# Dokumushikun/jittor-clip-fewshot

Hardware: AMD Instinct MI355X
Metric: images/sec ViT-B/32 fwd+LoRA-bwd bs=256 (higher is better)
Workload: dtype f32; 1 GPU; cfg-2: ViT-B/32 + rank-4 LoRA(q,k,v; 12 text + 12 vision blocks; shipped lora_weights.pkl) + 4 text-prompt tokens; run_lora train step = text tower fwd+bwd on 403 captions + image tower fwd+bwd + 100*cos CE + AdamW; global_batch=256, images_per_rank=256, captions=403, tower_streams=2, text_positions=77, parallelism=dp1

## Files before the change

### include/clipfs.h

```cpp
#ifndef CLIPFS_H
#define CLIPFS_H

#include <stddef.h>
#include <stdint.h>

#ifdef __cplusplus
extern "C" {
#endif

#define CLIPFS_OK 0
#define CLIPFS_EINVAL 1
#define CLIPFS_HIPERR_BASE 1000

#define CLIPFS_ABI_VERSION 2
int clipfs_abi_version(void);
const char* clipfs_source_stamp(void);
const char* clipfs_gemm_source_stamp(void);
const char* clipfs_last_error(void);

typedef struct clipfs_gemm_args {
  size_t struct_size;
  const float* A;
  const float* B;
  float* C;
  int M, N, K;
  int lda, ldb, ldc;
  float alpha;
  const float* bias;
  const float* residual;
  int ldres;
  int act;
  float* aux_out;
  const float* aux_in;
  const float* lora_t;
  const float* lora_b;
  int lora_r, lora_nseg, lora_seg_width;
  float lora_scale;
  int a_mode;
  int img_res, patch, out_tokens;
  const void* B_planes;
  int b_format;
  float* workspace;
  size_t workspace_floats;
  const void* A_f16;
  void* C_f16;
  int aux_f16;
  int* counters;
  size_t counters_ints;
} clipfs_gemm_args;
int clipfs_gemm_nt(const clipfs_gemm_args* args, void* stream);
int clipfs_split_bf16(const float* src, void* planes, size_t n, void* stream);
int clipfs_convert_f16(const float* src, void* dst, size_t n, void* stream);
int clipfs_gemm_splits(int M, int N, int K);
int clipfs_gemm_tile_rows(int M, int N);
#define CLIPFS_F16_64X128 0
#define CLIPFS_F16_64X128_S2 1
#define CLIPFS_F16_128X128 2
#define CLIPFS_F16_256X128 3
#define CLIPFS_F16_PP_REG 4
#define CLIPFS_F16_PP_LDS 5
#define CLIPFS_F16_PH16 6
#define CLIPFS_F16_PH16_WIDE 7
#define CLIPFS_F16_PH32 8
typedef struct clipfs_f16_launch {
  int kernel;
  int m_begin, m_end;
  int side;
} clipfs_f16_launch;
typedef struct clipfs_f16_plan {
  int n;
  clipfs_f16_launch launch[3];
} clipfs_f16_plan;
int clipfs_gemm_f16_plan(const clipfs_gemm_args* args, int cus, clipfs_f16_plan* out);
size_t clipfs_gemm_workspace_floats(int M, int N, int K);
size_t clipfs_gemm_counter_ints(int M, int N, int K);
int clipfs_gemm_timing(int enable);
int clipfs_gemm_timing_collect(double* total_ms, double* total_flops, int* launches);
double clipfs_gemm_timing_last_bytes(void);

int clipfs_layernorm_fwd(const float* x, int ldx, const float* gamma, const float* beta, float* y,
                         float* mean, float* rstd, int rows, int width, float eps, void* stream);
int clipfs_layernorm_bwd(const float* dy, const float* x, int ldx, const float* gamma, const float* mean,
                         const float* rstd, const float* dres, float* dx, int lddx, int rows, int width,
                         void* stream);
int clipfs_layernorm_bwd_rows(const float* dy, const float* x, int ldx, const float* gamma, const float* mean,
                              const float* rstd, const int32_t* xmap, const float* dres, float* dx, int lddx, int rows,
                              int width, void* stream);
int clipfs_layernorm_fwd_f16(const float* x, int ldx, const float* gamma, const float* beta, float* y, void* y16,
                             float* mean, float* rstd, int rows, int width, float eps, void* stream);
int clipfs_layernorm_bwd_f16(const float* dy, const float* x, int ldx, const float* gamma, const float* mean,
                             const float* rstd, const float* dres, float* dx, void* dx16, int lddx, int rows, int width,
                             void* stream);
int clipfs_layernorm_bwd_rows_f16(const float* dy, const float* x, int ldx, const float* gamma, const float* mean,
                                  const float* rstd, const int32_t* xmap, const float* dres, float* dx, void* dx16, int lddx,
                                  int rows, int width, void* stream);
int clipfs_layernorm_fwd_lora_ok(int width, int r, int nseg);
int clipfs_layernorm_fwd_lora(const float* x, int ldx, const float* gamma, const float* beta, float* y, void* y16,
                              float* mean, float* rstd, int rows, int width, float eps, const float* A, float* t, int r,
                              int nseg, unsigned seg_mask, float p, uint64_t seed, uint32_t stream_base, uint32_t drow0,
                              void* keep_bits, void* stream);
int clipfs_layernorm_fwd_lora_map(const float* x, int ldx, const float* gamma, const float* beta, float* y, void* y16,
                                  float* mean, float* rstd, int rows, int width, float eps, const float* A, float* t, int r,
                                  int nseg, unsigned seg_mask, float p, uint64_t seed, uint32_t stream_base, uint32_t drow0,
                                  const int32_t* drow_map, void* keep_bits, void* stream);

int clipfs_attention_fwd(const float* qkv, float* out, float* lse, int batch, int seq, int heads, int causal,
                         void* stream);
// ... 256 lines not shown
```

### jittor-clip-fewshot_amd/clipfs/_lib.py

```python
from __future__ import annotations

import ctypes as C
import os

ABI_VERSION = 2

_HERE = os.path.dirname(os.path.abspath(__file__))
_TAG = os.environ.get("CLIPFS_LIB_TAG", "")
LIB_PATH = os.path.join(_HERE, f"libclipfs_hip_{_TAG}.so" if _TAG else "libclipfs_hip.so")

c_f32p = C.c_void_p
c_stream = C.c_void_p


class ClipfsError(RuntimeError):
    pass


class GemmArgs(C.Structure):
    _fields_ = [
        ("struct_size", C.c_size_t),
        ("A", C.c_void_p), ("B", C.c_void_p), ("C", C.c_void_p),
        ("M", C.c_int), ("N", C.c_int), ("K", C.c_int),
        ("lda", C.c_int), ("ldb", C.c_int), ("ldc", C.c_int),
# ... 39 lines not shown
    _fields_ = [("family", C.c_int), ("groups", C.c_int), ("rq", C.c_int), ("sr_b", C.c_int), ("slices_b", C.c_int),
                ("sr_a", C.c_int), ("slices_a", C.c_int), ("work_floats", C.c_size_t), ("part_a_offset", C.c_size_t),
                ("keep_bits_ok", C.c_int), ("f16dy_ok", C.c_int), ("launches", C.c_int), ("launch", LoraLaunch * 6)]


LORA_OPS = ("down", "bwd", "bwd_f16dy")
LORA_X_ACT, LORA_KEEP_BITS, LORA_FROZEN, LORA_DX = 1, 2, 4, 8
LORA_FAMILIES = ("mfma", "row")

F16_KERNELS = ("64x128", "64x128_s2", "128x128", "256x128", "pp_reg", "pp_lds", "ph16", "ph16_wide", "ph32")


class Block(C.Structure):
    _fields_ = [(n, C.c_void_p) for n in (
        "ln1_g", "ln1_b", "ln2_g", "ln2_b",
        "w_qkv", "b_qkv", "w_qkv_t",
        "w_o", "b_o", "w_o_t",
        "w_fc", "b_fc", "w_fc_t",
        "w_pr", "b_pr", "w_pr_t",
        "lora_a_qkv", "lora_b_qkv", "lora_a_o", "lora_b_o",
        "g_lora_a_qkv", "g_lora_b_qkv", "g_lora_a_o", "g_lora_b_o")] + [("lora_mask", C.c_uint)] + [
        (n, C.c_void_p) for n in ("w_qkv_p", "w_o_p", "w_fc_p", "w_pr_p", "w_qkv_t_p", "w_o_t_p", "w_fc_t_p", "w_pr_t_p",
                                  "g_ln1_b", "g_ln2_b", "g_b_q", "g_b_k", "g_b_v", "g_b_o", "g_b_fc", "g_b_pr",
                                  "lora_a_fc", "lora_b_fc", "lora_a_pr", "lora_b_pr",
                                  "g_lora_a_fc", "g_lora_b_fc", "g_lora_a_pr", "g_lora_b_pr",
                                  "prompt", "g_prompt")] + [("prompt_first", C.c_int), ("prompt_rows", C.c_int)]


class Tower(C.Structure):
    _fields_ = [
        ("struct_size", C.c_size_t), ("block_size", C.c_size_t),
        ("width", C.c_int), ("heads", C.c_int), ("layers", C.c_int), ("seq", C.c_int), ("causal", C.c_int),
        ("lora_r", C.c_int), ("lora_scale", C.c_float), ("lora_dropout", C.c_float),
        ("dropout_seed", C.c_uint64), ("dropout_stream0", C.c_uint32), ("dropout_row0", C.c_uint32),
        ("blocks", C.POINTER(Block)), ("weight_format", C.c_int),
        ("gemm_counters", C.c_void_p), ("gemm_counters_ints", C.c_size_t),
        ("grad_lo", C.c_int),
    ]


_i, _f, _p, _sz = C.c_int, C.c_float, C.c_void_p, C.c_size_t
_u, _u64, _u32 = C.c_uint, C.c_uint64, C.c_uint32

SIGNATURES = {
    "clipfs_abi_version": (_i, []),
    "clipfs_last_error": (C.c_char_p, []),
    "clipfs_source_stamp": (C.c_char_p, []),
    "clipfs_gemm_source_stamp": (C.c_char_p, []),
    "clipfs_gemm_nt": (_i, [C.POINTER(GemmArgs), _p]),
    "clipfs_split_bf16": (_i, [_p, _p, _sz, _p]),
    "clipfs_convert_f16": (_i, [_p, _p, _sz, _p]),
    "clipfs_gemm_splits": (_i, [_i, _i, _i]),
    "clipfs_gemm_tile_rows": (_i, [_i, _i]),
    "clipfs_gemm_f16_plan": (_i, [C.POINTER(GemmArgs), _i, C.POINTER(F16Plan)]),
    "clipfs_gemm_workspace_floats": (_sz, [_i, _i, _i]),
    "clipfs_gemm_counter_ints": (_sz, [_i, _i, _i]),
    "clipfs_gemm_timing": (_i, [_i]),
    "clipfs_gemm_timing_collect": (_i, [C.POINTER(C.c_double), C.POINTER(C.c_double), C.POINTER(C.c_int)]),
    "clipfs_gemm_timing_last_bytes": (C.c_double, []),
    "clipfs_layernorm_fwd": (_i, [_p, _i, _p, _p, _p, _p, _p, _i, _i, _f, _p]),
    "clipfs_layernorm_bwd": (_i, [_p, _p, _i, _p, _p, _p, _p, _p, _i, _i, _i, _p]),
    "clipfs_layernorm_fwd_f16": (_i, [_p, _i, _p, _p, _p, _p, _p, _p, _i, _i, _f, _p]),
    "clipfs_layernorm_fwd_lora_ok": (_i, [_i, _i, _i]),
    "clipfs_layernorm_fwd_lora": (_i, [_p, _i, _p, _p, _p, _p, _p, _p, _i, _i, _f, _p, _p, _i, _i, _u, _f, _u64, _u32, _u32, _p, _p]),
    "clipfs_layernorm_bwd_f16": (_i, [_p, _p, _i, _p, _p, _p, _p, _p, _p, _i, _i, _i, _p]),
    "clipfs_attention_fwd": (_i, [_p, _p, _p, _i, _i, _i, _i, _p]),
    "clipfs_attention_bwd": (_i, [_p, _p, _p, _p, _p, _p, _i, _i, _i, _i, _p]),
    "clipfs_attention_lse_floats": (_sz, [_i, _i, _i]),
    "clipfs_attention_plan": (_i, [_i, _i, _i, _i, _i, _i, C.POINTER(AttentionPlan)]),
    "clipfs_attention_mfma_max_seq": (_i, []),
    "clipfs_attention_mfma_long_fwd": (_i, [_p, _p, _p, _i, _i, _i, _i, _i, _i, _p]),
    "clipfs_attention_mfma_long_bwd": (_i, [_p, _p, _p, _p, _p, _p, _i, _i, _i, _i, _i, _i, _p]),
    "clipfs_attention_f16_max_seq": (_i, []),
    "clipfs_attention_f16_fwd": (_i, [_p, _i, _p, _p, _p, _i, _i, _i, _i, _p]),
    "clipfs_attention_f16_bwd": (_i, [_p, _i, _p, _i, _p, _p, _p, _p, _p, _i, _i, _i, _i, _p]),
    "clipfs_lora_keep_bits_ok": (_i, [_i, _i, _i, _i]),
    "clipfs_lora_plan": (_i, [_i, _i, _i, _i, _i, _i, _i, C.POINTER(LoraPlan)]),
    "clipfs_lora_down": (_i, [_p, _p, _p, _i, _i, _i, _i, _u, _f, _u64, _u32, _u32, _p, _p]),
    "clipfs_lora_bwd_work_floats": (_sz, [_i, _i, _i, _i]),
    "clipfs_lora_bwd": (_i, [_p, _p, _p, _p, _p, _p, _p, _p, _p, _i, _i, _i, _i, _i, _u, _f, _f, _u64, _u32, _u32, _p, _p, _p]),
    "clipfs_lora_bwd_work_floats2": (_sz, [_i, _i, _i, _i, _i]),
    "clipfs_lora_bwd_xact": (_i, [_p, _p, _p, _p, _p, _p, _p, _p, _p, _i, _i, _i, _i, _f, _f, _u64, _u32, _u32, _i, _p, _p]),
    "clipfs_gelu_bwd_inplace": (_i, [_p, _p, _sz, _p]),
    "clipfs_lora_bwd_f16dy_ok": (_i, [_i, _i, _i, _i]),
    "clipfs_lora_bwd_f16dy": (_i, [_p, _p, _p, _p, _p, _p, _p, _p, _p, _i, _i, _i, _i, _i, _u, _f, _f, _u64, _u32, _u32, _p, _p, _p]),
    "clipfs_vit_fill_special": (_i, [_p, _p, _p, _p, _i, _i, _i, _i, _i, _p]),
    "clipfs_text_embed": (_i, [_p, _p, _p, _p, _i, _p, _i, _i, _i, _p]),
    "clipfs_token_rows_grad": (_i, [_p, _p, _i, _i, _i, _i, _i, _p]),
    "clipfs_matmul_small": (_i, [_p, _p, _p, _i, _i, _i, C.c_long, C.c_long, C.c_long, C.c_long, _f, _p]),
    "clipfs_gather_eot": (_i, [_p, _p, _p, _p, _i, _i, _i, _p]),
    "clipfs_scatter_rows": (_i, [_p, _p, _p, _i, _i, _i, _p]),
    "clipfs_gather_seq_rows": (_i, [_p, _sz, _p, _p, _i, _i, _i, _p]),
    "clipfs_add_seq_rows": (_i, [_p, _p, _p, _i, _i, _i, _p]),
    "clipfs_put_seq_rows": (_i, [_p, _p, _p, _sz, _i, _i, _i, _p]),
    "clipfs_eot_index": (_i, [_p, _p, _i, _i, _p]),
    "clipfs_gather_seq_rows_f16": (_i, [_p, _sz, _p, _p, _i, _i, _i, _p]),
    "clipfs_put_seq_rows_f16": (_i, [_p, _p, _p, _sz, _i, _i, _i, _p]),
    "clipfs_l2norm_fwd": (_i, [_p, _p, _p, _i, _i, _p]),
    "clipfs_l2norm_bwd": (_i, [_p, _p, _p, _p, _i, _i, _p]),
    "clipfs_class_mean_fwd": (_i, [_p, _p, _i, _i, _i, _p]),
    "clipfs_class_mean_bwd": (_i, [_p, _p, _p, _i, _i, _i, _p]),
    "clipfs_cross_entropy": (_i, [_p, _p, _p, _p, _p, _p, _i, _i, _f, _p]),
    "clipfs_topk": (_i, [_p, _p, _i, _i, _i, _p]),
    "clipfs_channel_affine": (_i, [_p, _p, _p, _p, _i, _i, _p]),
    "clipfs_logit_normalize": (_i, [_p, _p, _p, _i, _i, _p]),
    "clipfs_logit_normalize_bwd": (_i, [_p, _p, _p, _i, _i, _p]),
# ... 126 lines not shown
```

### jittor-clip-fewshot_amd/csrc/gemm.hip

```cpp
#include "common.h"
#include "gemm_common.h"

#include <stdlib.h>

#include <vector>

#ifdef CLIPFS_ABLATION_BUILD
#define CLIPFS_ABLATE(mask, bit) ((mask) & (bit))
#else
#define CLIPFS_ABLATE(mask, bit) 0
#endif

#ifdef CLIPFS_STAMPS
__device__ unsigned long long clipfs_gemm_stamps[16384 * 6];
#define CLIPFS_STAMP(i)                                                                                     \
  do {                                                                                                      \
    if (threadIdx.x == 0 && blockIdx.x < 16384) {                                                           \
      clipfs_gemm_stamps[blockIdx.x * 6 + (i)] = __builtin_amdgcn_s_memtime();                              \
      if ((i) == 1) clipfs_gemm_stamps[blockIdx.x * 6 + 4] = __builtin_amdgcn_s_memrealtime();              \
      if ((i) == 2) clipfs_gemm_stamps[blockIdx.x * 6 + 5] = __builtin_amdgcn_s_memrealtime();              \
      if (0) {                                                                                       \
        unsigned hw, xcc;                                                                                   \
        asm volatile("s_getreg_b32 %0, hwreg(HW_REG_HW_ID)" : "=s"(hw));                                  \
        asm volatile("s_getreg_b32 %0, hwreg(HW_REG_XCC_ID)" : "=s"(xcc));                                \
        clipfs_gemm_stamps[blockIdx.x * 6 + 4] = hw;                                                        \
        clipfs_gemm_stamps[blockIdx.x * 6 + 5] = xcc;                                                       \
      }                                                                                                     \
    }                                                                                                       \
  } while (0)
extern "C" int clipfs_debug_read_stamps(unsigned long long* host, int n) {
  return (int)hipMemcpyFromSymbol(host, HIP_SYMBOL(clipfs_gemm_stamps), sizeof(unsigned long long) * n, 0, hipMemcpyDeviceToHost);
}
#else
#define CLIPFS_STAMP(i) do {} while (0)
#endif

namespace clipfs {

typedef float f32x16 __attribute__((ext_vector_type(16)));
typedef float f32x4 __attribute__((ext_vector_type(4)));
typedef unsigned int u32x4v __attribute__((ext_vector_type(4)));

__device__ __forceinline__ void glds16(const float* gsrc, float* lds_wave_base) {
  __builtin_amdgcn_global_load_lds((const __attribute__((address_space(1))) void*)gsrc,
                                   (__attribute__((address_space(3))) void*)lds_wave_base, 16, 0, 0);
}

template <int BM, int BN, int AMODE>
__global__ __launch_bounds__(256) void gemm_nt_kernel(const GemmParams p) {
  extern __shared__ __attribute__((aligned(16))) float smem[];
  constexpr int WM = BM >= 64 ? 2 : 1;
  constexpr int WN = 4 / WM;
  constexpr int TM = BM / (32 * WM);
  constexpr int TN = BN / (32 * WN);
  constexpr int A_CHUNKS = BM * 8 / 256;
  constexpr int B_CHUNKS = BN * 8 / 256;
  constexpr int STAGE_FLOATS = (BM + BN) * BK;

  const clipfs_gemm_args& g = p.a;
  CLIPFS_STAMP(0);
  const int tid = threadIdx.x;
  const int lane = tid & 63;
  const int wave = tid >> 6;
  const int wm = wave / WN, wn = wave % WN;
  int tile;
  {
    const int nwg = gridDim.x, bid = blockIdx.x;
    const int xcd = bid & 7, li = bid >> 3, q = nwg >> 3, r = nwg & 7;
    tile = (xcd < r ? xcd * (q + 1) : r * (q + 1) + (xcd - r) * q) + li;
  }
  const int split = tile % p.splits;
  tile /= p.splits;
  const int GM = p.gm;
  const int nbn = p.n_blocks_n;
  const int grp = tile / (GM * nbn);
  const int rem = tile - grp * (GM * nbn);
  const int mb_total = (g.M + BM - 1) / BM;
  const int gm = min(GM, mb_total - grp * GM);
  const int m0 = (grp * GM + rem % gm) * BM;
  const int n0 = (rem / gm) * BN;
  const int M = g.M, N = g.N, K = g.K;

  const float* a_src[A_CHUNKS];
  int a_lds[A_CHUNKS];
  const int kc = tid & 7;
#pragma unroll
  for (int i = 0; i < A_CHUNKS; ++i) {
    const int row = (tid >> 3) + 32 * i;
    const int m = min(m0 + row, M - 1);
    if (AMODE == 0 || AMODE == 3 || (AMODE == 2 && g.a_mode == 0)) {
      a_src[i] = g.A + (size_t)m * g.lda + (AMODE == 0 ? kc * 4 : 0);
    } else {
      const int b = m / p.patches, pp = m - b * p.patches;
      const int py = pp / p.grid_g, px = pp - py * p.grid_g;
      a_src[i] = g.A + ((size_t)b * 3 * g.img_res + (size_t)py * g.patch) * g.img_res + (size_t)px * g.patch +
                 (AMODE == 1 ? kc * 4 : 0);
    }
    a_lds[i] = row * BK + ((kc ^ ((row >> 1) & 7)) << 2);
  }
  const float* b_src[B_CHUNKS];
  int b_lds[B_CHUNKS];
#pragma unroll
  for (int i = 0; i < B_CHUNKS; ++i) {
    const int row = (tid >> 3) + 32 * i;
    const int n = min(n0 + row, N - 1);
    b_src[i] = g.B + (size_t)n * g.ldb + (AMODE != 2 ? kc * 4 : 0);
    b_lds[i] = BM * BK + row * BK + ((kc ^ ((row >> 1) & 7)) << 2);
  }

  f32x4 a_reg[A_CHUNKS], b_reg[B_CHUNKS];
  auto load_global = [&](int kt) __attribute__((always_inline)) {
    if (AMODE == 0 || AMODE == 3) {
      const int k0 = kt * BK;
#pragma unroll
      for (int i = 0; i < A_CHUNKS; ++i) a_reg[i] = *reinterpret_cast<const f32x4*>(a_src[i] + k0);
#pragma unroll
      for (int i = 0; i < B_CHUNKS; ++i) b_reg[i] = *reinterpret_cast<const f32x4*>(b_src[i] + k0);
    } else if (AMODE == 1) {
      const int k0 = kt * BK;
      const size_t off = ((size_t)(kt >> 5) * g.img_res + (kt & 31)) * g.img_res;
#pragma unroll
      for (int i = 0; i < A_CHUNKS; ++i) a_reg[i] = *reinterpret_cast<const f32x4*>(a_src[i] + off);
#pragma unroll
      for (int i = 0; i < B_CHUNKS; ++i) b_reg[i] = *reinterpret_cast<const f32x4*>(b_src[i] + k0);
    } else {
      const int k = kt * BK + kc * 4;
      const bool k_ok = k < K;
      if (g.a_mode == 0) {
#pragma unroll
        for (int i = 0; i < A_CHUNKS; ++i)
          a_reg[i] = k_ok ? *reinterpret_cast<const f32x4*>(a_src[i] + k) : f32x4{0.f, 0.f, 0.f, 0.f};
      } else {
        const int pp2 = g.patch * g.patch;
// ... 125 lines not shown
    {
      const auto rs = __builtin_amdgcn_make_buffer_rsrc(p.part + ((size_t)tile * S + split) * SLAB, 0, SLAB * 4, 0x00020000);
#pragma unroll
      for (int i = 0; i < TM; ++i)
#pragma unroll
        for (int j = 0; j < TN; ++j)
#pragma unroll
          for (int v = 0; v < 4; ++v) {
            const f32x4 val = f32x4{acc[i][j][4 * v], acc[i][j][4 * v + 1], acc[i][j][4 * v + 2], acc[i][j][4 * v + 3]};
            __builtin_amdgcn_raw_buffer_store_b128(__builtin_bit_cast(u32x4v, val), rs,
                                                   (((i * TN + j) * 4 + v) * 256 + tid) * 16, 0,  16);
          }
    }
    int* flag = reinterpret_cast<int*>(smem + 2 * STAGE_FLOATS);
    asm volatile("s_waitcnt vmcnt(0)" ::: "memory");
    __syncthreads();
    if (tid == 0) {
      const int old = __hip_atomic_fetch_add(p.sk_cnt + tile, 1, __ATOMIC_RELAXED, __HIP_MEMORY_SCOPE_AGENT);
      const int last = old == S - 1;
      if (last) __hip_atomic_store(p.sk_cnt + tile, 0, __ATOMIC_RELAXED, __HIP_MEMORY_SCOPE_AGENT);
      *flag = last;
    }
    __syncthreads();
    if (!*flag) return;
    if (S > 2) {
#pragma unroll
      for (int i = 0; i < TM; ++i)
#pragma unroll
        for (int j = 0; j < TN; ++j)
#pragma unroll
          for (int r = 0; r < 16; ++r) acc[i][j][r] = 0.f;
    }
    for (int c = 0; c < S; ++c) {
      if (S == 2 && c == split) continue;
      const auto rs = __builtin_amdgcn_make_buffer_rsrc(p.part + ((size_t)tile * S + c) * SLAB, 0, SLAB * 4, 0x00020000);
#pragma unroll
      for (int i = 0; i < TM; ++i)
#pragma unroll
        for (int j = 0; j < TN; ++j) {
          f32x4 u[4];
#pragma unroll
          for (int v = 0; v < 4; ++v)
            u[v] = __builtin_bit_cast(f32x4, __builtin_amdgcn_raw_buffer_load_b128(
                                                 rs, (((i * TN + j) * 4 + v) * 256 + tid) * 16, 0,  16));
#pragma unroll
          for (int v = 0; v < 4; ++v)
#pragma unroll
            for (int e = 0; e < 4; ++e) acc[i][j][4 * v + e] += u[v][e];
        }
    }
  }
  finish_tiles<TM, TN>(g, p.patches, acc, m0 + wm * (BM / WM), n0 + wn * (BN / WN), m0 + BM <= M && n0 + BN <= N, lane);
  CLIPFS_STAMP(3);
}

struct SkSeg {
  int tile, kb, ke;
};

#ifndef CLIPFS_SK_WAVES
#define CLIPFS_SK_WAVES 2
#endif
template <int BM, int BN, int NSTAGE>
__global__ __launch_bounds__(256, CLIPFS_SK_WAVES) void gemm_sk_kernel(const GemmParams p) {
  extern __shared__ __attribute__((aligned(16))) float smem[];
  constexpr int WM = BM >= 64 ? 2 : 1;
  constexpr int WN = 4 / WM;
  constexpr int TM = BM / (32 * WM);
  constexpr int TN = BN / (32 * WN);
  constexpr int A_CHUNKS = BM * 8 / 256;
  constexpr int B_CHUNKS = BN * 8 / 256;
  constexpr int STAGE_FLOATS = (BM + BN) * BK;
  constexpr int SLAB_BYTES = BM * BN * 4;

  const clipfs_gemm_args& g = p.a;
  const int tid = threadIdx.x;
  const int lane = tid & 63;
  const int wave = tid >> 6;
  const int uw = __builtin_amdgcn_readfirstlane(wave);
  const int wm = wave / WN, wn = wave % WN;
  const int M = g.M, N = g.N;
  const int nk = p.sk_nk;
  const int runs = gridDim.x;
  const int w = xcd_contiguous_unit();
  int* flag = reinterpret_cast<int*>(smem + NSTAGE * STAGE_FLOATS);

  const int q = p.sk_q, r = p.sk_r;
  const int sk_it0 = w * q + min(w, r);
  const int sk_it1 = sk_it0 + q + (w < r ? 1 : 0);
  const int rpx = runs >> 3;
  const int xcd = rpx > 0 ? w / rpx : 0, li = rpx > 0 ? w - xcd * rpx : 0;
  struct Cursor {
    int it, rd;
  };
  auto next_seg = [&](Cursor& c, SkSeg& sg) -> bool {
    if (c.it < sk_it1) {
      const int t = c.it / nk;
      sg.tile = p.sk_tile0 + t;
      sg.kb = c.it - t * nk;
      sg.ke = min(nk, sg.kb + (sk_it1 - c.it));
      c.it += sg.ke - sg.kb;
      return true;
    }
    if (c.rd < p.sk_dp_rounds) {
      sg.tile = (xcd * p.sk_dp_rounds + c.rd) * rpx + li;
      sg.kb = 0;
// ... 192 lines not shown
      if (tid == 0) {
        const int old = __hip_atomic_fetch_add(p.sk_cnt + cur.tile, 1, __ATOMIC_RELAXED, __HIP_MEMORY_SCOPE_AGENT);
        const int last = old == nc - 1;
        if (last) __hip_atomic_store(p.sk_cnt + cur.tile, 0, __ATOMIC_RELAXED, __HIP_MEMORY_SCOPE_AGENT);
        *flag = last;
      }
      __syncthreads();
      if (*flag) {
        if (nc > 2) {
#pragma unroll
          for (int i = 0; i < TM; ++i)
#pragma unroll
            for (int j = 0; j < TN; ++j)
#pragma unroll
              for (int rr = 0; rr < 16; ++rr) acc[i][j][rr] = 0.f;
        }
        for (int c = w_lo; c <= w_hi; ++c) {
          if (nc == 2 && c == w) continue;
          const int ckind = begin_of(c) > t_lo_it ? 0 : 1;
          const auto rs = __builtin_amdgcn_make_buffer_rsrc(p.sk_part + ((size_t)(2 * c + ckind)) * (BM * BN), 0, SLAB_BYTES,
                                                           0x00020000);
#pragma unroll
          for (int i = 0; i < TM; ++i)
#pragma unroll
            for (int j = 0; j < TN; ++j) {
              f32x4 u[4];
#pragma unroll
              for (int v = 0; v < 4; ++v)
                u[v] = __builtin_bit_cast(f32x4, __builtin_amdgcn_raw_buffer_load_b128(
                                                     rs, (((i * TN + j) * 4 + v) * 256 + tid) * 16, 0,  16));
#pragma unroll
              for (int v = 0; v < 4; ++v)
#pragma unroll
                for (int e = 0; e < 4; ++e) acc[i][j][4 * v + e] += u[v][e];
            }
        }
        finish_tiles<TM, TN>(g, p.patches, acc, mw, nw, full_tile, lane);
      }
    }
    cur = nxt;
    have = have_n;
  }
}

struct TimedLaunch {
  hipEvent_t start, stop;
  double flops;
  double bytes;
};
static thread_local double g_last_bytes = 0.0;
static thread_local bool g_timing = false;
static thread_local std::vector<TimedLaunch>* g_timed = nullptr;

template <int BM, int BN, int AMODE>
static int launch(const GemmParams& p, hipStream_t stream) {
  const int mb = (p.a.M + BM - 1) / BM;
  static const int lds_pad = getenv("CLIPFS_GEMM_LDS_PAD") ? atoi(getenv("CLIPFS_GEMM_LDS_PAD")) : 8;
  const size_t lds = 2 * (size_t)(BM + BN) * BK * sizeof(float) + (size_t)lds_pad * 1024 + 64;
  static bool attr_set = false;
  if (!attr_set && lds > 48 * 1024) {
    (void)hipFuncSetAttribute(reinterpret_cast<const void*>(&gemm_nt_kernel<BM, BN, AMODE>),
                        hipFuncAttributeMaxDynamicSharedMemorySize, (int)lds);
    attr_set = true;
  }
  hipLaunchKernelGGL((gemm_nt_kernel<BM, BN, AMODE>), dim3(mb * p.n_blocks_n * p.splits), dim3(256), lds, stream, p);
  return launch_status();
}

static int cu_count() {
  static int n = 0;
  if (!n) {
    int dev = 0, v = 0;
    if (hipGetDevice(&dev) == hipSuccess &&
        hipDeviceGetAttribute(&v, hipDeviceAttributeMultiprocessorCount, dev) == hipSuccess && v > 0)
      n = v;
    else
      n = 256;
  }
  return n;
}

constexpr int SK_MIN_STEPS = 8;

struct SkConfig {
  bool use;
  int per_cu;
};

static inline int sk_env(const char* name, int dflt) {
  const char* v = getenv(name);
  return v ? atoi(v) : dflt;
}

static inline SkConfig sk_config(int M, int N, int K) {
  static const int mode = sk_env("CLIPFS_GEMM_SK", 0);
  static const int per_cu = sk_env("CLIPFS_GEMM_SK_PER_CU", 2);
  SkConfig c;
  c.per_cu = per_cu > 0 ? per_cu : 2;
  const long tiles = (long)((M + 63) / 64) * ((N + 127) / 128);
  const int nk = K / BK;
  const long slots = (long)cu_count() * c.per_cu;
  c.use = mode == 2 || (mode == 1 && (nk >= 24 || (tiles < 2 * slots && tiles * nk >= 2L * SK_MIN_STEPS * 64)));
  return c;
}

struct SkPlan {
  int runs, dp_rounds, tile0, sk_tiles, q, r;
};

static inline SkPlan sk_plan(long tiles, int nk, int per_cu) {
  SkPlan s;
  const long slots = (long)cu_count() * per_cu;
  long runs = tiles * nk / SK_MIN_STEPS;
  if (runs < tiles) runs = tiles;
  if (runs > slots) runs = slots;
  if (runs > tiles * nk) runs = tiles * nk;
  s.runs = (int)(runs < 1 ? 1 : runs);
  s.dp_rounds = 0;
  if ((s.runs & 7) == 0 && tiles >= 2L * s.runs) s.dp_rounds = (int)(tiles / s.runs) - 1;
  s.tile0 = s.dp_rounds * s.runs;
  s.sk_tiles = (int)(tiles - s.tile0);
  const long iters = (long)s.sk_tiles * nk;
  s.q = (int)(iters / s.runs);
  s.r = (int)(iters % s.runs);
  return s;
}

template <int BM, int BN, int NSTAGE>
static int launch_sk(GemmParams& p, int per_cu, hipStream_t stream) {
  const int mb = (p.a.M + BM - 1) / BM;
  p.n_blocks_n = (p.a.N + BN - 1) / BN;
  p.sk_nk = p.a.K / BK;
  const SkPlan s = sk_plan((long)mb * p.n_blocks_n, p.sk_nk, per_cu);
  p.sk_tile0 = s.tile0;
  p.sk_dp_rounds = s.dp_rounds;
  p.sk_q = s.q;
  p.sk_r = s.r;
  p.sk_part = p.a.workspace;
  p.sk_cnt = p.a.counters;
  size_t lds = NSTAGE * (size_t)(BM + BN) * BK * sizeof(float) + 64;
  const size_t want = (size_t)(160 * 1024 / (per_cu + 1)) + 1024;
  if (lds < want && want * per_cu <= 160 * 1024) lds = want;
  static size_t attr_lds = 0;
  if (lds > attr_lds && lds > 48 * 1024) {
    (void)hipFuncSetAttribute(reinterpret_cast<const void*>(&gemm_sk_kernel<BM, BN, NSTAGE>),
                              hipFuncAttributeMaxDynamicSharedMemorySize, (int)lds);
    attr_lds = lds;
  }
  hipLaunchKernelGGL((gemm_sk_kernel<BM, BN, NSTAGE>), dim3(s.runs), dim3(256), lds, stream, p);
  return launch_status();
}

}

using namespace clipfs;

static inline int gemm_bm(int M, int N) {
  static const int force = getenv("CLIPFS_GEMM_BM") ? atoi(getenv("CLIPFS_GEMM_BM")) : 0;
  if (force == 32 || force == 64) return force;
  const long nbn = (N + 127) / 128;
  const long t64 = (long)((M + 63) / 64) * nbn, t32 = (long)((M + 31) / 32) * nbn;
  const double cost64 = (double)((t64 + 255) / 256) * 64.0, cost32 = (double)((t32 + 255) / 256) * 32.0 * 1.08;
  return cost32 < cost64 ? 32 : 64;
}

extern "C" int clipfs_gemm_tile_rows(int M, int N) { return gemm_bm(M, N); }

extern "C" int clipfs_gemm_splits(int M, int N, int K) {
  if (M <= 0 || N <= 0 || K <= 0) return 1;
  static const int force = getenv("CLIPFS_GEMM_SPLITS") ? atoi(getenv("CLIPFS_GEMM_SPLITS")) : 0;
  if (force > 0) return (K + BK - 1) / BK >= 2 * force ? force : 1;
  const int bm = gemm_bm(M, N);
  const long tiles = (long)((M + bm - 1) / bm) * ((N + 127) / 128);
  const int nk = (K + BK - 1) / BK;
  if (tiles >= 384 || nk < 8) return 1;
  long s = (448 + tiles - 1) / tiles;
  if (s > nk / 4) s = nk / 4;
  if (s > 8) s = 8;
  return s < 1 ? 1 : (int)s;
}

static inline long splitk_tiles(int M, int N, int K) {
  if (clipfs_gemm_splits(M, N, K) <= 1) return 0;
  const int bm = gemm_bm(M, N);
  return (long)((M + bm - 1) / bm) * ((N + 127) / 128);
}

static inline bool sk_enabled() {
  static const bool on = sk_env("CLIPFS_GEMM_SK", 0) != 0;
  return on;
}

static inline void sk_geometry(int M, int N, int K, long* tiles, size_t* slab_floats) {
  const SkConfig c = sk_config(M, N, K);
  *tiles = (long)((M + 63) / 64) * ((N + 127) / 128);
  *slab_floats = c.use ? (size_t)2 * sk_plan(*tiles, K / BK, c.per_cu).runs * 64 * 128 : 0;
}

extern "C" size_t clipfs_gemm_workspace_floats(int M, int N, int K) {
  if (M <= 0 || N <= 0 || K <= 0) return 0;
  const int s = clipfs_gemm_splits(M, N, K);
  size_t need = s > 1 ? (size_t)s * (size_t)splitk_tiles(M, N, K) * gemm_bm(M, N) * 128 : 0;
  if (sk_enabled() && (K % BK) == 0) {
    long tiles;
    size_t sk;
    sk_geometry(M, N, K, &tiles, &sk);
    need = sk > need ? sk : need;
  }
  return need;
}

extern "C" size_t clipfs_gemm_counter_ints(int M, int N, int K) {
  if (M <= 0 || N <= 0 || K <= 0) return 0;
  size_t need = (size_t)splitk_tiles(M, N, K);
  if (sk_enabled() && (K % BK) == 0) {
    long tiles;
    size_t slab;
    sk_geometry(M, N, K, &tiles, &slab);
    if (slab && (size_t)tiles > need) need = (size_t)tiles;
// ... 90 lines not shown
  return rc;
}

static int gemm_nt_impl(const clipfs_gemm_args* args, void* stream) {
  CLIPFS_REQUIRE(args != nullptr, "gemm: null args");
  const clipfs_gemm_args& a = *args;
  CLIPFS_REQUIRE(a.struct_size == sizeof(clipfs_gemm_args),
                 "gemm: args built against another clipfs.h (struct_size %zu, library has %zu)", a.struct_size,
                 sizeof(clipfs_gemm_args));
  CLIPFS_REQUIRE(a.M > 0 && a.N > 0 && a.K > 0, "gemm: bad dims %d %d %d", a.M, a.N, a.K);
  if (a.A_f16) {
    CLIPFS_CHECK(gemm_f16_validate(a));
    return gemm_f16_dispatch(a, (hipStream_t)stream);
  }
  CLIPFS_REQUIRE(!a.C_f16 && !a.aux_f16, "gemm: C_f16 / aux_f16 belong to the f16 x f16 kernel only");
  CLIPFS_REQUIRE(a.A && a.B && a.C, "gemm: null operand");
  CLIPFS_REQUIRE((a.K & 3) == 0 && (a.ldb & 3) == 0 && aligned16(a.B), "gemm: K and ldb must be multiples of 4, B 16-byte aligned");
  CLIPFS_REQUIRE(a.ldb >= a.K && a.ldc >= a.N, "gemm: leading dimension too small");
  CLIPFS_REQUIRE(a.act >= 0 && a.act <= 3, "gemm: bad act %d", a.act);
  CLIPFS_REQUIRE(a.act != 3 || !a.B_planes, "gemm: act 3 (ReLU) belongs to the exact fp32 kernels");
  CLIPFS_REQUIRE(a.act != 2 || a.aux_in, "gemm: act 2 needs aux_in");
  CLIPFS_REQUIRE(!a.residual || a.ldres >= a.N, "gemm: ldres too small");
  GemmParams p;
  p.a = a;
  p.patches = 0;
#ifdef CLIPFS_ABLATION_BUILD
  static const int ablate_cfg = getenv("CLIPFS_GEMM_ABLATE") ? atoi(getenv("CLIPFS_GEMM_ABLATE")) : 0;
  p.ablate = ablate_cfg;
#else
  p.ablate = 0;
#endif
  p.grid_g = 0;
  static const int gm_cfg = getenv("CLIPFS_GEMM_GM") ? atoi(getenv("CLIPFS_GEMM_GM")) : 8;
  p.gm = gm_cfg > 0 ? gm_cfg : 8;
  if (a.a_mode == 0) {
    CLIPFS_REQUIRE((a.lda & 3) == 0 && a.lda >= a.K && aligned16(a.A), "gemm: lda must be a multiple of 4 and >= K, A 16-byte aligned");
  } else {
    CLIPFS_REQUIRE(a.a_mode == 1, "gemm: bad a_mode %d", a.a_mode);
    CLIPFS_REQUIRE(a.patch > 0 && a.img_res % a.patch == 0, "gemm: image %d not divisible by patch %d", a.img_res, a.patch);
    p.grid_g = a.img_res / a.patch;
    p.patches = p.grid_g * p.grid_g;
    CLIPFS_REQUIRE(a.K == 3 * a.patch * a.patch, "gemm: patch mode needs K == 3*patch^2");
    CLIPFS_REQUIRE(a.M % p.patches == 0 && a.out_tokens >= p.patches + 1, "gemm: patch mode shape mismatch");
    CLIPFS_REQUIRE((a.patch & 3) != 0 || ((a.img_res & 3) == 0 && aligned16(a.A)), "gemm: image rows must be 16-byte aligned");
  }
  if (a.lora_t) {
    CLIPFS_REQUIRE(a.lora_b && a.lora_r > 0 && a.lora_nseg > 0 && a.lora_seg_width > 0, "gemm: bad lora args");
    CLIPFS_REQUIRE(a.lora_seg_width % 32 == 0 && a.lora_seg_width * a.lora_nseg >= a.N, "gemm: lora segment width must be a multiple of 32 and cover N");
  }
  hipStream_t s = (hipStream_t)stream;
  p.splits = 1;
  p.part = nullptr;
  p.n_blocks_n = 0;
  if (a.B_planes && (a.b_format == 1 || a.b_format == 2) && a.a_mode == 0 && (a.K % BK) == 0 && a.ldb == a.K)
    return gemm_bf16x3_dispatch(p, s);
  p.sk_cnt = nullptr;
  {
    const int want = clipfs_gemm_splits(a.M, a.N, a.K);
    if (want > 1 && a.a_mode == 0 && (a.K % BK) == 0 && a.workspace && a.counters && aligned16(a.workspace) &&
        a.workspace_floats >= clipfs_gemm_workspace_floats(a.M, a.N, a.K) &&
        a.counters_ints >= (size_t)splitk_tiles(a.M, a.N, a.K)) {
      p.splits = want;
      p.part = a.workspace;
      p.sk_cnt = a.counters;
    }
  }
  static const int tile_cfg = getenv("CLIPFS_GEMM_TILE") ? atoi(getenv("CLIPFS_GEMM_TILE")) : 0;
  if (tile_cfg == 1 && a.a_mode == 0 && (a.K % BK) == 0) {
    p.splits = 1;
    p.n_blocks_n = (a.N + 127) / 128;
    return launch<128, 128, 3>(p, s);
  }
  if (tile_cfg == 2 && a.a_mode == 0 && (a.K % BK) == 0) {
    p.splits = 1;
    p.n_blocks_n = (a.N + 63) / 64;
    return launch<128, 64, 0>(p, s);
  }
  if (sk_enabled() && tile_cfg == 0 && a.a_mode == 0 && (a.K % BK) == 0 && a.workspace && a.counters &&
      sk_config(a.M, a.N, a.K).use &&
      (long)((a.M + 63) / 64) * ((a.N + 127) / 128) * 2 * (a.K / BK) < (1L << 30) &&
      a.workspace_floats >= clipfs_gemm_workspace_floats(a.M, a.N, a.K) &&
      a.counters_ints >= clipfs_gemm_counter_ints(a.M, a.N, a.K)) {
    CLIPFS_REQUIRE(aligned16(a.workspace), "gemm: workspace must be 16-byte aligned");
    p.splits = 1;
    return launch_sk<64, 128, 2>(p, sk_config(a.M, a.N, a.K).per_cu, s);
  }
  p.n_blocks_n = (a.N + 127) / 128;
  if (gemm_bm(a.M, a.N) == 32 && a.a_mode == 0 && (a.K % BK) == 0) return launch<32, 128, 3>(p, s);
  static const int glds_cfg = getenv("CLIPFS_GEMM_GLDS") ? atoi(getenv("CLIPFS_GEMM_GLDS")) : 1;
  if (a.a_mode == 0 && (a.K % BK) == 0) return glds_cfg ? launch<64, 128, 3>(p, s) : launch<64, 128, 0>(p, s);
  if (a.a_mode == 1 && a.patch == 32 && (a.img_res & 3) == 0) return launch<64, 128, 1>(p, s);
  return launch<64, 128, 2>(p, s);
}
```

### jittor-clip-fewshot_amd/csrc/gemm_common.h

```cpp
#pragma once
#include "common.h"

namespace clipfs {

typedef float f32x16 __attribute__((ext_vector_type(16)));

struct GemmParams {
  clipfs_gemm_args a;
  int n_blocks_n;
  int patches;
  int grid_g;
  int splits;
  float* part;
  int gm;
  int ablate;
  int sk_nk;
  int sk_tile0;
  int sk_dp_rounds;
  int sk_q, sk_r;
  float* sk_part;
  int* sk_cnt;
};

constexpr int BK = 32;

__device__ __forceinline__ void epilogue_store(const clipfs_gemm_args& g, int patches, int m, int n, float accv,
                                               bool lora_done = false) {
  float v = g.alpha * accv + (g.bias ? g.bias[n] : 0.f);
  if (g.lora_t && !lora_done) {
    const int lseg = n / g.lora_seg_width;
    const float* lb = g.lora_b + (size_t)n * g.lora_r;
    const float* t = g.lora_t + (size_t)m * (g.lora_nseg * g.lora_r) + lseg * g.lora_r;
    float d = 0.f;
    for (int jj = 0; jj < g.lora_r; ++jj) d = fmaf(t[jj], lb[jj], d);
    v = fmaf(g.lora_scale, d, v);
  }
  size_t orow = (size_t)m, rrow = (size_t)m;
  if (g.a_mode == 1) {
    const int b = m / patches, pp = m - b * patches;
    orow = (size_t)b * g.out_tokens + 1 + pp;
    rrow = (size_t)(1 + pp);
  }
  if (g.act == 1) {
    if (g.aux_out) g.aux_out[orow * g.ldc + n] = v;
    v = quick_gelu(v);
  } else if (g.act == 2) {
    v *= quick_gelu_grad(g.aux_in[orow * g.ldc + n]);
  }
  if (g.residual) v += g.residual[rrow * g.ldres + n];
  if (g.act == 3) v = fmaxf(v, 0.f);
  g.C[orow * g.ldc + n] = v;
}


template <int TM, int TN>
__device__ __forceinline__ void finish_tiles(const clipfs_gemm_args& g, int patches, f32x16 (&acc)[TM][TN], int mw, int nw,
                                             bool full_tile, int lane) {
  const int fr = lane & 31, fh = lane >> 5;
  const int M = g.M, N = g.N;
  const bool lora_mfma = g.lora_t && g.alpha == 1.f;
  if (lora_mfma) {
    const int r = g.lora_r, tw = g.lora_nseg * r;
    const int rsteps = (r + 1) >> 1;
    for (int st = 0; st < rsteps; ++st) {
      const int k = 2 * st + fh;
      const float kmask = k < r ? 1.f : 0.f;
      const int kc2 = min(k, r - 1);
      float bv[TN];
      int segs[TN];
#pragma unroll
      for (int j = 0; j < TN; ++j) {
        const int nb = nw + j * 32;
        segs[j] = min(nb, N - 1) / g.lora_seg_width;
        bv[j] = g.lora_b[(size_t)min(nb + fr, N - 1) * r + kc2] * kmask;
// ... 100 lines not shown
```

Before: 4871 images/s.

## Add mixed 64/32-row tile GEMM kernel to reduce wave quantization

Measured after the change: 4928 images/s, median of 6. 1.01x the previous value.

```diff
diff --git a/include/clipfs.h b/include/clipfs.h
--- a/include/clipfs.h
+++ b/include/clipfs.h
@@ -53,6 +53,7 @@
 int clipfs_convert_f16(const float* src, void* dst, size_t n, void* stream);
 int clipfs_gemm_splits(int M, int N, int K);
 int clipfs_gemm_tile_rows(int M, int N);
+int clipfs_gemm_mixed_rows64(int M, int N, int K);
 #define CLIPFS_F16_64X128 0
 #define CLIPFS_F16_64X128_S2 1
 #define CLIPFS_F16_128X128 2
diff --git a/jittor-clip-fewshot_amd/clipfs/_lib.py b/jittor-clip-fewshot_amd/clipfs/_lib.py
--- a/jittor-clip-fewshot_amd/clipfs/_lib.py
+++ b/jittor-clip-fewshot_amd/clipfs/_lib.py
@@ -115,6 +115,7 @@
     "clipfs_convert_f16": (_i, [_p, _p, _sz, _p]),
     "clipfs_gemm_splits": (_i, [_i, _i, _i]),
     "clipfs_gemm_tile_rows": (_i, [_i, _i]),
+    "clipfs_gemm_mixed_rows64": (_i, [_i, _i, _i]),
     "clipfs_gemm_f16_plan": (_i, [C.POINTER(GemmArgs), _i, C.POINTER(F16Plan)]),
     "clipfs_gemm_workspace_floats": (_sz, [_i, _i, _i]),
     "clipfs_gemm_counter_ints": (_sz, [_i, _i, _i]),
diff --git a/jittor-clip-fewshot_amd/csrc/gemm.hip b/jittor-clip-fewshot_amd/csrc/gemm.hip
--- a/jittor-clip-fewshot_amd/csrc/gemm.hip
+++ b/jittor-clip-fewshot_amd/csrc/gemm.hip
@@ -47,7 +47,7 @@
 }
 
 template <int BM, int BN, int AMODE>
-__global__ __launch_bounds__(256) void gemm_nt_kernel(const GemmParams p) {
+__device__ __forceinline__ void gemm_nt_tile(const GemmParams& p, const int tile, const int split, const int m0, const int n0) {
   extern __shared__ __attribute__((aligned(16))) float smem[];
   constexpr int WM = BM >= 64 ? 2 : 1;
   constexpr int WN = 4 / WM;
@@ -63,22 +63,6 @@
   const int lane = tid & 63;
   const int wave = tid >> 6;
   const int wm = wave / WN, wn = wave % WN;
-  int tile;
-  {
-    const int nwg = gridDim.x, bid = blockIdx.x;
-    const int xcd = bid & 7, li = bid >> 3, q = nwg >> 3, r = nwg & 7;
-    tile = (xcd < r ? xcd * (q + 1) : r * (q + 1) + (xcd - r) * q) + li;
-  }
-  const int split = tile % p.splits;
-  tile /= p.splits;
-  const int GM = p.gm;
-  const int nbn = p.n_blocks_n;
-  const int grp = tile / (GM * nbn);
-  const int rem = tile - grp * (GM * nbn);
-  const int mb_total = (g.M + BM - 1) / BM;
-  const int gm = min(GM, mb_total - grp * GM);
-  const int m0 = (grp * GM + rem % gm) * BM;
-  const int n0 = (rem / gm) * BN;
   const int M = g.M, N = g.N, K = g.K;
 
   const float* a_src[A_CHUNKS];
@@ -310,6 +294,41 @@
   }
   finish_tiles<TM, TN>(g, p.patches, acc, m0 + wm * (BM / WM), n0 + wn * (BN / WN), m0 + BM <= M && n0 + BN <= N, lane);
   CLIPFS_STAMP(3);
+}
+
+__device__ __forceinline__ int xcd_contiguous(int bid, int nwg) {
+  const int xcd = bid & 7, li = bid >> 3, q = nwg >> 3, r = nwg & 7;
+  return (xcd < r ? xcd * (q + 1) : r * (q + 1) + (xcd - r) * q) + li;
+}
+
+__device__ __forceinline__ void tile_blocks(int tile, int GM, int nbn, int mb_total, int& mb, int& nb) {
+  const int grp = tile / (GM * nbn);
+  const int rem = tile - grp * (GM * nbn);
+  const int gm = min(GM, mb_total - grp * GM);
+  mb = grp * GM + rem % gm;
+  nb = rem / gm;
+}
+
+template <int BM, int BN, int AMODE>
+__global__ __launch_bounds__(256) void gemm_nt_kernel(const GemmParams p) {
+  int tile = xcd_contiguous(blockIdx.x, gridDim.x);
+  const int split = tile % p.splits;
+  tile /= p.splits;
+  int mb, nb;
+  tile_blocks(tile, p.gm, p.n_blocks_n, (p.a.M + BM - 1) / BM, mb, nb);
+  gemm_nt_tile<BM, BN, AMODE>(p, tile, split, mb * BM, nb * BN);
+}
+
+__global__ __launch_bounds__(256) void gemm_nt_mixed_kernel(const GemmParams p) {
+  const int bid = blockIdx.x, t64 = p.mix_tiles64;
+  int mb, nb;
+  if (bid < t64) {
+    tile_blocks(xcd_contiguous(bid, t64), p.gm, p.n_blocks_n, p.mix_rows64 / 64, mb, nb);
+    gemm_nt_tile<64, 128, 3>(p, 0, 0, mb * 64, nb * 128);
+  } else {
+    tile_blocks(xcd_contiguous(bid - t64, gridDim.x - t64), p.gm, p.n_blocks_n, (p.a.M - p.mix_rows64 + 31) / 32, mb, nb);
+    gemm_nt_tile<32, 128, 3>(p, 0, 0, p.mix_rows64 + mb * 32, nb * 128);
+  }
 }
 
 struct SkSeg {
@@ -608,19 +627,32 @@
 static thread_local bool g_timing = false;
 static thread_local std::vector<TimedLaunch>* g_timed = nullptr;
 
+static size_t gemm_lds_bytes(int BM, int BN) {
+  static const int lds_pad = getenv("CLIPFS_GEMM_LDS_PAD") ? atoi(getenv("CLIPFS_GEMM_LDS_PAD")) : 8;
+  return 2 * (size_t)(BM + BN) * BK * sizeof(float) + (size_t)lds_pad * 1024 + 64;
+}
+
+template <typename Kernel>
+static int launch_kernel(Kernel kernel, bool& attr_set, unsigned grid, size_t lds, const GemmParams& p, hipStream_t stream) {
+  if (!attr_set && lds > 48 * 1024) {
+    (void)hipFuncSetAttribute(reinterpret_cast<const void*>(kernel), hipFuncAttributeMaxDynamicSharedMemorySize, (int)lds);
+    attr_set = true;
+  }
+  hipLaunchKernelGGL(kernel, dim3(grid), dim3(256), lds, stream, p);
+  return launch_status();
+}
+
 template <int BM, int BN, int AMODE>
 static int launch(const GemmParams& p, hipStream_t stream) {
+  static bool attr_set = false;
   const int mb = (p.a.M + BM - 1) / BM;
-  static const int lds_pad = getenv("CLIPFS_GEMM_LDS_PAD") ? atoi(getenv("CLIPFS_GEMM_LDS_PAD")) : 8;
-  const size_t lds = 2 * (size_t)(BM + BN) * BK * sizeof(float) + (size_t)lds_pad * 1024 + 64;
+  return launch_kernel(&gemm_nt_kernel<BM, BN, AMODE>, attr_set, (unsigned)(mb * p.n_blocks_n * p.splits), gemm_lds_bytes(BM, BN), p, stream);
+}
+
+static int launch_mixed(const GemmParams& p, hipStream_t stream) {
   static bool attr_set = false;
-  if (!attr_set && lds > 48 * 1024) {
-    (void)hipFuncSetAttribute(reinterpret_cast<const void*>(&gemm_nt_kernel<BM, BN, AMODE>),
-                        hipFuncAttributeMaxDynamicSharedMemorySize, (int)lds);
-    attr_set = true;
-  }
-  hipLaunchKernelGGL((gemm_nt_kernel<BM, BN, AMODE>), dim3(mb * p.n_blocks_n * p.splits), dim3(256), lds, stream, p);
-  return launch_status();
+  const int mb32 = (p.a.M - p.mix_rows64 + 31) / 32;
+  return launch_kernel(&gemm_nt_mixed_kernel, attr_set, (unsigned)(p.mix_tiles64 + mb32 * p.n_blocks_n), gemm_lds_bytes(64, 128), p, stream);
 }
 
 static int cu_count() {
@@ -721,6 +753,21 @@
 }
 
 extern "C" int clipfs_gemm_tile_rows(int M, int N) { return gemm_bm(M, N); }
+
+constexpr int BAND_MIN_M = 4096;
+
+static inline int gemm_mixed_rows64(int M, int N, int K) {
+  if (M < BAND_MIN_M || N <= 0 || K <= 0 || (K % BK) != 0 || gemm_bm(M, N) != 32 || clipfs_gemm_splits(M, N, K) > 1) return 0;
+  const long nbn = (N + 127) / 128;
+  const long rounds = (long)(M / 64) * nbn / 512;
+  const long mb64 = rounds * 512 / nbn;
+  const long t32 = ((M - mb64 * 64 + 31) / 32) * nbn;
+  const double cost_mix = (double)((mb64 * nbn + 255) / 256) * 64.0 + (double)((t32 + 255) / 256) * 32.0 * 1.08;
+  const double cost32 = (double)(((long)((M + 31) / 32) * nbn + 255) / 256) * 32.0 * 1.08;
+  return mb64 > 0 && cost_mix < cost32 ? (int)(mb64 * 64) : 0;
+}
+
+extern "C" int clipfs_gemm_mixed_rows64(int M, int N, int K) { return gemm_mixed_rows64(M, N, K); }
 
 extern "C" int clipfs_gemm_splits(int M, int N, int K) {
   if (M <= 0 || N <= 0 || K <= 0) return 1;
@@ -917,6 +964,7 @@
   p.splits = 1;
   p.part = nullptr;
   p.n_blocks_n = 0;
+  p.mix_rows64 = p.mix_tiles64 = 0;
   if (a.B_planes && (a.b_format == 1 || a.b_format == 2) && a.a_mode == 0 && (a.K % BK) == 0 && a.ldb == a.K)
     return gemm_bf16x3_dispatch(p, s);
   p.sk_cnt = nullptr;
@@ -951,8 +999,13 @@
     return launch_sk<64, 128, 2>(p, sk_config(a.M, a.N, a.K).per_cu, s);
   }
   p.n_blocks_n = (a.N + 127) / 128;
+  static const int glds_cfg = getenv("CLIPFS_GEMM_GLDS") ? atoi(getenv("CLIPFS_GEMM_GLDS")) : 1;
+  if (a.a_mode == 0 && p.splits == 1 && glds_cfg) {
+    p.mix_rows64 = gemm_mixed_rows64(a.M, a.N, a.K);
+    p.mix_tiles64 = p.mix_rows64 / 64 * p.n_blocks_n;
+    if (p.mix_rows64 > 0) return launch_mixed(p, s);
+  }
   if (gemm_bm(a.M, a.N) == 32 && a.a_mode == 0 && (a.K % BK) == 0) return launch<32, 128, 3>(p, s);
-  static const int glds_cfg = getenv("CLIPFS_GEMM_GLDS") ? atoi(getenv("CLIPFS_GEMM_GLDS")) : 1;
   if (a.a_mode == 0 && (a.K % BK) == 0) return glds_cfg ? launch<64, 128, 3>(p, s) : launch<64, 128, 0>(p, s);
   if (a.a_mode == 1 && a.patch == 32 && (a.img_res & 3) == 0) return launch<64, 128, 1>(p, s);
   return launch<64, 128, 2>(p, s);
diff --git a/jittor-clip-fewshot_amd/csrc/gemm_common.h b/jittor-clip-fewshot_amd/csrc/gemm_common.h
--- a/jittor-clip-fewshot_amd/csrc/gemm_common.h
+++ b/jittor-clip-fewshot_amd/csrc/gemm_common.h
@@ -20,6 +20,7 @@
   int sk_q, sk_r;
   float* sk_part;
   int* sk_cnt;
+  int mix_rows64, mix_tiles64;
 };
 
 constexpr int BK = 32;
```
